# tavildar/Polar

Hardware: AMD Instinct MI355X
Metric: codewords/s (N=2048 K=1024 L=32 LLR-SCL) (higher is better)
Workload: dtype f64

## Files before the change

### polar_amd/__init__.py

```python
import ctypes as C
import os

import numpy as np

try:
    import torch
except Exception:
    torch = None

_HERE = os.path.dirname(os.path.abspath(__file__))
LIB_PATH = os.environ.get("POLAR_AMD_LIB") or os.path.join(_HERE, "libpolar_amd.so")

_dp = C.POINTER(C.c_double)
_u8p = C.POINTER(C.c_uint8)
_u16p = C.POINTER(C.c_uint16)
_u64p = C.POINTER(C.c_uint64)


ASK4_GRAY, ASK8_GRAY, ASK16_GRAY, BPSK = 1, 2, 3, 4
ASK4_SP, ASK8_SP, ASK16_SP = 5, 6, 7
CONSTELLATION_NAMES = {"bpsk": BPSK, "ask4-gray": ASK4_GRAY, "ask8-gray": ASK8_GRAY, "ask16-gray": ASK16_GRAY,
                       "ask4-sp": ASK4_SP, "ask8-sp": ASK8_SP, "ask16-sp": ASK16_SP}
_NBITS = {BPSK: 1, ASK4_GRAY: 2, ASK4_SP: 2, ASK8_GRAY: 3, ASK8_SP: 3, ASK16_GRAY: 4, ASK16_SP: 4}
RX_MLC = 0x100
# ... 203 lines not shown
            if n == -1:
                return None
            if n < 0:
                raise PolarError(f"polar_debug_mc_alive: HIP status {-n - 1}")
            a = np.zeros(max(n, 1), np.uint64)
            if int(f(self._h, which, _p(a, _u64p), n)) != n:
                raise PolarError("polar_debug_mc_alive: the count changed between two reads")
            lists.append(np.sort(a[:n]))
        return tuple(lists)

    def debug_ctl_words(self, marked=True):
        f = self._L.polar_debug_ctl_words
        f.restype = C.c_long
        f.argtypes = [C.c_void_p, C.POINTER(C.c_uint32), C.c_long, C.c_int]
        words = np.zeros(self.N, np.uint32)
        n = int(f(self._h, _p(words, C.POINTER(C.c_uint32)), self.N, 1 if marked else 0))
        if n != self.N:
            raise PolarError(f"polar_debug_ctl_words: {n}")
        return words

    @classmethod
    def from_block_length(cls, block_length, info_length, design_epsilon, crc_size=0):
        n = int(round(np.log2(block_length)))
        if (1 << n) != block_length:
            raise PolarError("block_length must be a power of two")
        return cls(n, info_length, design_epsilon, crc_size)

    @classmethod
    def from_tables(cls, num_layers, info_length, crc_size, frozen, order, crc_matrix=None):
        frozen = np.ascontiguousarray(frozen, np.uint8)
        order = np.ascontiguousarray(order, np.uint16)
# ... 760 lines not shown
```

### polar_amd/build.py

```python
import os
import shutil
import subprocess
import sys

HERE = os.path.dirname(os.path.abspath(__file__))
ROOT = os.path.dirname(HERE)
CSRC = os.path.join(HERE, "csrc")
INC = os.path.join(ROOT, "include")
LIB = os.path.join(HERE, "libpolar_amd.so")
BUILD = os.path.join(HERE, "_build")
FLAGS_LIST32 = ["-mllvm", "-amdgpu-sched-strategy=max-memory-clause", "-mllvm", "-amdgpu-use-amdgpu-trackers"] + \
               os.environ.get("POLAR_LIST32_FLAGS", "").split()
FLAGS_LAT = os.environ.get("POLAR_LAT_FLAGS", "").split()
SOURCES = [("polar_kernels.hip", ["POLAR_ED_TU=0"], "", []), ("polar_kernels.hip", ["POLAR_ED_TU=1"], ".ed", []),
           ("polar_kernels.hip", ["POLAR_ED_TU=2"], ".ed32", FLAGS_LIST32), ("polar_kernels.hip", ["POLAR_ED_TU=3"], ".lat", FLAGS_LAT),
           ("polar_kernels.hip", ["POLAR_ED_TU=4"], ".list", []),
           ("polar_kernels.hip", ["POLAR_ED_TU=5"], ".headA", []), ("polar_kernels.hip", ["POLAR_ED_TU=6"], ".headB", FLAGS_LIST32),
           ("polar_kernels.hip", ["POLAR_ED_TU=7"], ".adapt", []),
           ("polar_kernels_sc.hip", [], "", []), ("polar_kernels_p1.hip", [], "", []), ("polar_channel.hip", [], "", []),
           ("polar_construct.hip", [], "", []), ("polar_kernels_mlc.hip", [], "", []), ("polar_kernels_ga.hip", [], "", []),
           ("polar_kernels_metric.hip", [], "", []), ("polar_kernels_adapt.hip", [], "", []),
           ("polar_kernels_flip.hip", [], "", [])] + \
          [(f, [], "", []) for f in ("polar_handle.cpp", "polar_decode.cpp", "polar_hostpipe.cpp", "polar_montecarlo.cpp", "polar_multi.cpp",
                                     "polar_debug.cpp", "polar_ga.cpp", "polar_bicm.cpp", "polar_list.cpp", "polar_mlc.cpp", "polar_adaptive.cpp", "polar_flip.cpp")]
TEST_HOOK_SOURCES = ("polar_montecarlo.cpp", "polar_debug.cpp")
TEST_HOOK_KERNEL_TAGS = (".ed32", ".headB")
LIB_TEST = os.path.join(HERE, "libpolar_amd_test.so")
KNOWN_DEFS = {"POLAR_MARGIN", "POLAR_SLOTHIST", "SCLAT_PROF", "POLAR_DEV_GS32", "POLAR_DEV_ONE", "POLAR_NO_FIXED_N",
              "POLAR_NO_GUARD_INT", "POLAR_NO_COLD_HINTS", "OCC", "ED_NR", "POLAR_R1_RANK", "POLAR_R1_CHAIN"}
ARCH = os.environ.get("POLAR_ARCH", "gfx950")
_flags_ok = {}


def _probe_flags(flags):
    key = tuple(flags)
    if key not in _flags_ok:
        import tempfile
        ok = list(flags)
        with tempfile.TemporaryDirectory() as d:
            src = os.path.join(d, "probe.hip")
            open(src, "w").write("#include <hip/hip_runtime.h>\n__global__ void probe_kernel() {}\n")
            pairs = [flags[i:i + 2] for i in range(0, len(flags), 2)]
            ok = []
            for pr in pairs:
# ... 171 lines not shown
```

### polar_amd/csrc/polar_debug.cpp

```cpp
#include "polar_multi.h"
#include "polar_amd_debug.h"
#ifdef POLAR_TEST_HOOKS
#include "polar_head_plan.h"
hipError_t polar_r1_counts_read_ed32(unsigned long long *out);
hipError_t polar_r1_counts_read_head(unsigned long long *out);
#endif

extern "C" {

int polar_debug_weak_leaves(const polar_code_t *h) { return polar_get_weak_leaves(h); }

int polar_debug_set(polar_code_t *h, const char *key, long value) {
    if (!h || !key) return fail(POLAR_E_ARG, "NULL argument");
    polar_code::Knobs &k = h->knobs;
    const std::string s(key);
    if (s == "mode_override") { if (value < -1 || value > 2) return fail(POLAR_E_ARG, "mode_override must be -1 (none), 0, 1 or 2"); k.mode_override = (int)value; }
    else if (s == "sc_no_fold") k.sc_no_fold = value != 0;
    else if (s == "no_tables") k.no_tables = value != 0;
    else if (s == "no_head") k.no_head = value != 0;
    else if (s == "no_r1") k.no_r1 = value != 0;
    else if (s == "head_min_b") { if (value < 0) return fail(POLAR_E_ARG, "head_min_b must be >= 0 (0 = default)"); k.head_min_b = value; }
    else if (s == "no_fuse_front") k.no_fuse_front = value != 0;
    else if (s == "no_prefix") h->prefix_on = (value == 0);
    else if (s == "no_rccl") { k.no_rccl = value != 0; multi_release(h, false); }
    else if (s == "force_rccl") { k.force_rccl = value != 0; multi_release(h, false); }
#ifdef POLAR_TEST_HOOKS
    else if (s == "host_fail_alloc") k.host_fail_alloc = value;
    else if (s == "share_device") { k.share_device = value != 0; multi_release(h, false); }
    else if (s == "fail_device") k.fail_device = (int)value;
    else if (s == "fail_collective") k.fail_collective = (int)value;
#endif
    else if (s == "lat_max_b") k.lat_max_b = value;
    else if (s == "lat_grid") { if (value < 0) return fail(POLAR_E_ARG, "lat_grid must be >= 0 (0 = default)"); k.lat_grid = value; }
    else if (s == "lane_grid") { if (value < 0) return fail(POLAR_E_ARG, "lane_grid must be >= 0 (0 = default)"); k.lane_grid = value; }
    else if (s == "list_chunk_cw") { if (value < 0) return fail(POLAR_E_ARG, "list_chunk_cw must be >= 0"); k.list_chunk_cw = value; }
// ... 40 lines not shown
        while (P < h->N && h->frozen[P]) ++P;
        const int Q = P >= 256 ? 256 : (P < 33 ? 0 : (P < 64 ? 64 : (P < 128 ? 128 : 256)));
        const HeadPlan hp = head_plan(h->frozen.data(), h->n, Q, std::min(P, Q), h->N / 2);
        if (hp.phi_h != h->last_head_phi) return -3;
        std::vector<unsigned long long> rows2((size_t)h->last_head_b * 4);
        const size_t pitch = hp.record_words() * sizeof(unsigned long long);
        if (hipMemcpy2D(rows2.data(), 32, h->d_head_rec.p + 2 * 4, pitch, 32, (size_t)h->last_head_b, hipMemcpyDeviceToHost) != hipSuccess) return -4;
        long bad = 0;
        for (long b = 0; b < h->last_head_b; ++b) {
            unsigned long long r[4];
            for (int a = 0; a < 4; ++a) r[a] = rows2[(size_t)b * 4 + a];
            bad += head_record_ok(hp, r) ? 0 : 1;
        }
        return bad;
    }
    if (s.compare(0, 3, "r1_") == 0) {
        static const char *const names[6] = {"r1_committed", "r1_discarded", "r1_rank_tried", "r1_rank_committed", "r1_chain_tried", "r1_chain_committed"};
        for (int i = 0; i < 6; ++i) {
            if (s != names[i]) continue;
            unsigned long long c[6] = {0, 0, 0, 0, 0, 0};
            if ((h->last_head_phi ? polar_r1_counts_read_head(c) : polar_r1_counts_read_ed32(c)) != hipSuccess) return -2;
            return (long)c[i];
        }
    }
#endif
    if (s == "last_rounds") return h->last_rounds;
    if (s == "last_round_max_per_device") return h->last_round_max_per_device;
    if (s == "worker_threads_started") return h->worker_threads_started;
    if (s.compare(0, 9, "round_us_") == 0) {
        if (h->round_us.empty()) return 0;
        std::vector<long> v(h->round_us);
        if (s == "round_us_count") return (long)v.size();
        if (s == "round_us_first") return v.front();
        std::sort(v.begin(), v.end());
        if (s == "round_us_min") return v.front();
// ... 33 lines not shown
    if (ensure_device(h, dg_)) return -1;
    unsigned int count = 0;
    hipError_t e = hipMemcpy(&count, h->d_nalive.p + which, sizeof count, hipMemcpyDeviceToHost);
    if (e == hipSuccess && (size_t)count > h->d_alive[which].cap) return -(long)hipErrorInvalidValue - 1;
    const long n = std::min<long>(count, cap);
    if (e == hipSuccess && out && n > 0) e = hipMemcpy(out, h->d_alive[which].p, (size_t)n * sizeof(uint64_t), hipMemcpyDeviceToHost);
    return e == hipSuccess ? (long)count : -(long)e - 1;
}

long polar_debug_ctl_words(polar_code_t *h, uint32_t *words, long cap, int marked) {
    if (!h) return -1;
    DevGuard dg_;
    if (ensure_device(h, dg_)) return -1;
    const long n = std::min<long>(h->N, cap);
    if (words && n > 0) {
        const hipError_t e = hipMemcpy(words, marked ? h->d_ctl_r1.p : h->d_ctl.p, (size_t)n * sizeof(uint32_t), hipMemcpyDeviceToHost);
        if (e != hipSuccess) return -(long)e - 1;
    }
    return h->N;
}

}
```

### polar_amd/csrc/polar_decode.cpp

```cpp
#include "polar_host.h"
#include "polar_head_plan.h"

namespace {

int effective_mode(const polar_code *h) { return h->knobs.mode_override >= 0 ? h->knobs.mode_override : h->mode; }
long lat_resident(const polar_code *h, int gs) {
    const size_t lds = polar_decode_lat_lds_bytes(h->N, gs, h->W);
    return lds <= h->lds_per_block ? (long)h->num_cu * std::min<long>(4, (long)(h->lds_per_block / lds)) : 0;
}
bool use_sc_lat(const polar_code *h, long B) {
    return h->n <= polar_sc_lat_max_log() && polar_sc_lat_lds_bytes(h->N, (int)h->sc_lat_ops.size()) <= h->lds_per_block &&
           h->knobs.lat_max_b >= 0 && B <= (h->knobs.lat_max_b ? h->knobs.lat_max_b : 2048);
}

struct Call {
    polar_code *h;
    const void *d_llr; int llr_fmt; long B; const unsigned int *n_dev; int L; uint8_t *d_out; double *d_pm;
    hipStream_t st; void *ev_start, *ev_stop; int phase; Deferred *deferred;
    BatchGeometry g; PolarDecodeParams p;
};

int batch_setup(polar_code *h, long B, int L, BatchGeometry &g) {
    if (!batch_geometry(h, B, L, true, g)) return fail(POLAR_E_ARG, "lds_log %d does not fit the LDS", g.lds_log);
    if ((size_t)g.grid * g.big * 64 + 64 > h->d_llr_scr.cap) {
// ... 203 lines not shown
    BatchGeometry gm = *std::max_element(g, g + n, [](const BatchGeometry &a, const BatchGeometry &b) { return a.grid < b.grid; });
    int rc;
    while ((rc = ensure_batch_scratch(h, gm)) == POLAR_E_NOMEM && gm.grid > gm.wpb) {
        (void)hipGetLastError();
        gm.grid = std::max(gm.wpb, (gm.grid / 2 / gm.wpb) * gm.wpb);
    }
    for (int s = 0; s < n && !rc; ++s) g[s].grid = std::min(g[s].grid, gm.grid);
    return rc;
}

void polar_host::base_params(const polar_code *h, int L, long B, PolarDecodeParams &p) {
    p.n = h->n; p.N = h->N; p.K = h->K; p.crc = h->crc; p.L = L; p.W = h->W; p.B = B;
    p.prefix_q = 0; p.prefix_len = 0; p.pre = nullptr;
    p.llr = nullptr; p.llr_fmt = POLAR_LLR_F64; p.p0 = nullptr; p.out = nullptr; p.pm_out = nullptr;
    p.frozen = h->d_frozen.p; p.info_rank = h->d_info_rank.p; p.crc_mask = h->d_crc_mask.p; p.tabs = h->d_tabs.p;
    p.ctl = h->knobs.no_r1 ? h->d_ctl.p : h->d_ctl_r1.p; p.work = h->d_work.p; p.llr_scr = h->d_llr_scr.p; p.c_scr = h->d_c_scr.p; p.hist_scr = h->d_hist_scr.p;
    p.flags = nullptr; p.cw_list = nullptr; p.cw_count = nullptr; p.n_dev = nullptr; p.tab_scr = nullptr; p.var_scr = nullptr;
}

void polar_host::fill_enc(const polar_code *h, PolarEncodeParams &p) {
    memset(&p, 0, sizeof p);
    p.n = h->n; p.N = h->N; p.K = h->K; p.crc = h->crc;
    p.order = h->d_order.p; p.crcm = h->d_crcm.p;
    p.stride = 1;
    p.info_block_div = 100;
}

int polar_host::decode_impl(polar_code *h, const void *d_llr, int llr_fmt, long B, const unsigned int *n_dev, int L, uint8_t *d_out,
                            double *d_pm, void *stream, void *ev_start, void *ev_stop, int phase, Deferred *deferred) {
    if (deferred) *deferred = Deferred::None;
    int rc = check_args(h && d_llr && d_out, L, B);
// ... 195 lines not shown
```

### polar_amd/csrc/polar_handle.cpp

```cpp
#include "polar_host.h"

namespace polar_host {

thread_local std::string g_err;

int fail(int code, const char *fmt, ...) {
    char buf[512];
    va_list ap;
    va_start(ap, fmt);
    vsnprintf(buf, sizeof buf, fmt, ap);
    va_end(ap);
    g_err = buf;
    return code;
}

std::atomic<unsigned long> g_allocs{0};

int usable_cpus() {
    int n = (int)std::thread::hardware_concurrency();
    cpu_set_t set;
    if (sched_getaffinity(0, sizeof set, &set) == 0) n = CPU_COUNT(&set);
    if (FILE *f = fopen("/sys/fs/cgroup/cpu.max", "r")) {
        char q[32]; long per = 0;
        if (fscanf(f, "%31s %ld", q, &per) == 2 && strcmp(q, "max") != 0 && per > 0) n = std::min<long>(n, std::max<long>(1, atol(q) / per));
// ... 133 lines not shown
        std::vector<int> tu((size_t)N + 1, 0);
        for (int i = 0; i < N; ++i) tu[i + 1] = tu[i] + (h->frozen[i] ? 0 : 1);
        auto rate1 = [&](int i0, int Z) {
            if (i0 + Z > N) return false;
            for (int i = i0; i < i0 + Z; ++i) {
                if (h->frozen[i] || (h->ctl[i] & 0x100u)) return false;
                if (i < i0 + Z - 1 && (tu[i] & 31) == 31) return false;
            }
            return true;
        };
        for (int i = 0; i < N; i += 4) {
            if ((i & 7) == 0 && rate1(i, 8)) { h->ctl_r1[i] |= 3u << 9; h->ctl_r1[i + 4] |= 2u << 9; i += 4; continue; }
            if (rate1(i, 4)) h->ctl_r1[i] |= 2u << 9;
        }
    }
    h->crc_mask.assign((size_t)crc * h->W, 0u);
    for (int i = 0; i < crc; ++i) {
        uint32_t *m = &h->crc_mask[(size_t)i * h->W];
        for (int j = 0; j < K; ++j)
            if (h->crcm[(size_t)i * K + j] & 1) m[h->info_rank[j] >> 5] ^= 1u << (h->info_rank[j] & 31);
        int r = h->info_rank[K + i];
        m[r >> 5] ^= 1u << (r & 31);
    }
    return POLAR_OK;
}

int ensure_device(polar_code *h, DevGuard &dg) {
    if (h->ctx_stuck) return fail(POLAR_E_DEVICE, "an earlier multi-device round of this handle never returned: the handle accepts no further calls (create a new one)");
    int cur = -1;
    if (hipGetDevice(&cur) == hipSuccess && h->device >= 0 && cur != h->device) dg.prev = cur;
// ... 7 lines not shown
        return fail(POLAR_E_DEVICE, "no HIP device available (%s); this library has no CPU decode path",
                    e == hipSuccess ? "device count 0" : hipGetErrorString(e));
    if (h->device < 0) HIP_TRY(hipGetDevice(&h->device));
    HIP_TRY(hipSetDevice(h->device));
    hipDeviceProp_t prop;
    HIP_TRY(hipGetDeviceProperties(&prop, h->device));
    h->num_cu = prop.multiProcessorCount;
    {
        int v = 0;
        h->lds_per_block = (hipDeviceGetAttribute(&v, hipDeviceAttributeMaxSharedMemoryPerBlock, h->device) == hipSuccess && v > 0) ? (size_t)v : (size_t)64 * 1024;
    }
    int rc;
    if ((rc = upload(h->d_frozen, h->frozen))) return rc;
    if ((rc = upload(h->d_ctl, h->ctl))) return rc;
    if ((rc = upload(h->d_ctl_r1, h->ctl_r1))) return rc;
    if ((rc = upload(h->d_sc_ops, h->sc_ops))) return rc;
    if ((rc = upload(h->d_sc_lat_ops, h->sc_lat_ops))) return rc;
    if ((rc = upload(h->d_order, h->order))) return rc;
    if ((rc = upload(h->d_info_rank, h->info_rank))) return rc;
    if ((rc = upload(h->d_crc_mask, h->crc_mask))) return rc;
    if ((rc = upload(h->d_crcm, h->crcm))) return rc;
    {
        std::vector<double> t(322);
        for (int j = 0; j < 64; ++j) t[j] = j ? 2.0 * std::exp2(-(double)(64 - j) / 64.0) : 1.0;
        for (int j = 0; j <= 128; ++j) {
            t[64 + j] = 1.0 / (1.0 + (double)j / 128.0);
            t[64 + 129 + j] = std::log1p((double)j / 128.0);
        }
        if ((rc = upload(h->d_tabs, t))) return rc;
    }
    h->dev_ready = true;
    return POLAR_OK;
}

int read_env_knobs(polar_code *h) {
    auto on = [](const char *name) { const char *e = getenv(name); return e && *e && strcmp(e, "0") != 0; };
    if (const char *e = getenv("POLAR_MODE")) {
        if (!(e[0] >= '0' && e[0] <= '2' && e[1] == 0)) return fail(POLAR_E_ARG, "POLAR_MODE=%s: must be 0, 1 or 2", e);
        h->knobs.mode_override = e[0] - '0';
    }
    h->knobs.sc_no_fold = on("POLAR_SC_NO_FOLD");
    h->knobs.no_tables = on("POLAR_NO_TABLES");
    h->knobs.no_head = on("POLAR_NO_HEAD");
    h->knobs.no_r1 = on("POLAR_NO_R1");
    h->knobs.no_rccl = on("POLAR_NO_RCCL");
    h->knobs.force_rccl = on("POLAR_FORCE_RCCL");
    return POLAR_OK;
}

void drop_clones(polar_code *h) {
    if (h->multi_poisoned) return;
    for (polar_code *c : h->clones) polar_destroy(c);
    h->clones.clear();
    if (h->hpipe) for (polar_code *&c : h->hpipe->ctx) if (c) { polar_destroy(c); c = nullptr; }
}

}

extern "C" {
// ... 61 lines not shown
}

void polar_destroy(polar_code_t *h) {
    if (!h) return;
    if (h->multi_poisoned) return;
    multi_release(h, false);
    for (polar_code *c : h->clones) polar_destroy(c);
    h->clones.clear();
    hostpipe_release(h);
    DevGuard dg_;
    {
        int cur = -1;
        if (h->dev_ready && hipGetDevice(&cur) == hipSuccess && cur != h->device) dg_.prev = cur;
    }
    if (h->dev_ready) (void)hipSetDevice(h->device);
    h->d_frozen.release(); h->d_ctl.release(); h->d_ctl_r1.release(); h->d_crcm.release(); h->d_order.release(); h->d_info_rank.release();
    h->d_crc_mask.release(); h->d_tabs.release(); h->d_pre.release(); h->d_llr_scr.release(); h->d_c_scr.release(); h->d_hist_scr.release();
    h->d_in.release(); h->d_f32.release(); h->d_out.release(); h->d_bytes_a.release(); h->d_bytes_b.release();
    h->d_counter.release(); h->d_sel.release(); h->d_work.release();
    h->d_ech.release(); h->d_flags.release(); h->d_list.release(); h->d_count.release(); h->d_bicm_llr.release(); h->d_list_out.release(); h->d_metric_scr.release(); h->d_adapt_ctl.release();
    h->d_alive[0].release(); h->d_alive[1].release(); h->d_nalive.release(); h->d_mc_ctr.release();
    for (auto &sl : h->mc_slots) { sl.list[0].release(); sl.list[1].release(); }
    h->d_slot_n.release();
    if (h->pin_in) (void)hipHostFree(h->pin_in);
    if (h->pin_out) (void)hipHostFree(h->pin_out);
    h->d_flip_ops.release(); h->d_flip_i32.release(); h->d_sc_ops.release(); h->d_sc_lat_ops.release(); h->d_flag_words.release(); h->d_var_scr.release(); h->d_tab_scr.release(); h->d_head_rec.release();
    delete h;
}

int polar_get_params(const polar_code_t *h, int *n, int *N, int *K, int *crc) {
    if (!h) return fail(POLAR_E_ARG, "NULL handle");
// ... 65 lines not shown
```

### polar_amd/csrc/polar_host.h

```cpp
#pragma once
#include <hip/hip_runtime.h>

#include <dlfcn.h>
#include <sched.h>
#include <sys/mman.h>
#include <unistd.h>

#include <algorithm>
#include <atomic>
#include <chrono>
#include <condition_variable>
#include <memory>
#include <mutex>
#include <thread>
#include <cmath>
#include <cstdarg>
#include <cstdio>
#include <cstdlib>
#include <cstring>
#include <functional>
#include <numeric>
#include <string>
#include <vector>

// ... 164 lines not shown
};

struct polar_code {
    int n = 0, N = 0, K = 0, crc = 0;
    double eps = 0.0;
    std::vector<uint8_t> frozen;
    std::vector<uint16_t> order;
    std::vector<uint16_t> bitrev;
    std::vector<uint8_t> crcm;
    int W = 0;
    std::vector<uint16_t> info_rank;
    std::vector<uint32_t> crc_mask;
    std::vector<uint8_t> sched;
    std::vector<uint32_t> ctl;
    std::vector<uint32_t> ctl_r1;
    int weak_leaves = 0;
    std::vector<uint32_t> sc_ops;
    std::vector<uint32_t> sc_lat_ops;
    bool sc_fold = false;
    bool dev_ready = false;
    int device = -1, num_cu = 0;
    size_t lds_per_block = 0;
    DevBuf<uint8_t> d_frozen, d_crcm;
    DevBuf<uint16_t> d_order, d_info_rank;
    DevBuf<uint32_t> d_crc_mask, d_ctl, d_ctl_r1, d_sc_ops, d_sc_lat_ops, d_var_scr;
    DevBuf<double> d_tab_scr;
    DevBuf<unsigned long long> d_head_rec;
    int last_head_phi = 0;
    long last_head_b = 0;
    long last_lat_waves = 0;
    long last_lane_waves = 0;
    const unsigned int *fb_count = nullptr;
    const uint32_t *fb_list = nullptr;
    void *fb_stream = nullptr;
    long fb_b = 0;
    void note_fallback(const unsigned int *count, const uint32_t *list, void *st, long B) { fb_count = count; fb_list = list; fb_stream = st; fb_b = B; }
    DevBuf<unsigned int> d_flag_words;
    DevBuf<double> d_llr_scr, d_tabs, d_pre;
    DevBuf<uint32_t> d_c_scr, d_hist_scr;
    DevBuf<double> d_in;
// ... 8 lines not shown
    DevBuf<unsigned int> d_count;
    DevBuf<double> d_list_out;
    DevBuf<double> d_metric_scr;
    DevBuf<unsigned int> d_adapt_ctl;
    std::vector<uint32_t> flip_ops;
    DevBuf<uint32_t> d_flip_ops;
    DevBuf<int32_t> d_flip_i32;
    DevBuf<double> d_bicm_llr;
    int mode = 0;
    struct Knobs {
        int mode_override = -1;
        bool sc_no_fold = false;
        bool no_tables = false;
        bool no_head = false;
        bool no_r1 = false;
        long head_min_b = 0;
        bool no_fuse_front = false;
        bool no_rccl = false;
        bool force_rccl = false;
        bool share_device = false;
        int fail_device = -1;
        int fail_collective = -1;
        long multi_timeout_s = 1800;
        long multi_grace_s = 10;
        bool force_workers = false;
        int stall_device = -1;
        long stall_ms = 0;
        long lat_max_b = 0;
        long host_pipe_min_bytes = 0;
        long host_chunk_bytes = 0;
// ... 136 lines not shown
```

### polar_amd/csrc/polar_kernels.hip

```cpp
#include <hip/hip_runtime.h>
#include <stdint.h>
#include <type_traits>

#include "polar_kernels.h"
#include "polar_device.h"
#include "polar_edom.h"

#ifdef POLAR_PROFILE
#define PROF_DECL u64 prof_acc[40] = {0,0,0,0,0,0,0,0,0,0,0,0,0,0,0,0,0,0,0,0,0,0,0,0,0,0,0,0,0,0,0,0,0,0,0,0,0,0,0,0}; u64 prof_t = __builtin_readcyclecounter();
#define PROF(i) { u64 t_ = __builtin_readcyclecounter(); prof_acc[i] += t_ - prof_t; prof_t = t_; }
#define PROF_OUT if (lane == 0 && p.pm_out) { for (int i_ = 0; i_ < 40; ++i_) atomicAdd((u64 *)p.pm_out + (i_ < 32 ? i_ : i_ + 2), prof_acc[i_]); }
#define PROF_CNT(i, v) { prof_acc[i] += (u64)(v); }
#define PROF_HEAD_DECL const int prof_head_phi = p.pm_out ? (int)((const u64 *)p.pm_out)[32] : 0; const u64 prof_head_t0 = prof_t; bool prof_head_open = prof_head_phi > 0;
#define PROF_HEAD(phi_) if (prof_head_open && (phi_) >= prof_head_phi) { prof_acc[22] += __builtin_readcyclecounter() - prof_head_t0; prof_head_open = false; }
#define PROF_HEAD_END prof_acc[23] += __builtin_readcyclecounter() - prof_head_t0;
#define PROF_R1_DECL int prof_r1_left = 0, prof_r1_slot = 24; bool prof_r1_open = false; u64 prof_r1_t0 = 0; \
                     const unsigned prof_r1_sw = p.pm_out ? (unsigned)((const u64 *)p.pm_out)[33] : 0u; \
                     const bool prof_r1_off = (prof_r1_sw & 1u) != 0, prof_rank_off = (prof_r1_sw & 2u) != 0, prof_chain_off = (prof_r1_sw & 4u) != 0; \
                     (void)prof_r1_off; (void)prof_rank_off; (void)prof_chain_off;
#define PROF_R1_ADD(d_) { if (prof_r1_slot == 24) prof_acc[24] += (d_); else if (prof_r1_slot == 32) prof_acc[32] += (d_); else prof_acc[34] += (d_); }
#define PROF_R1_TOP { if (prof_r1_open) { PROF_R1_ADD(prof_t - prof_r1_t0) prof_r1_open = false; } \
                      if (prof_r1_left > 0) { prof_r1_t0 = prof_t; prof_r1_open = true; --prof_r1_left; } }
#define PROF_R1_LEAF(ctl_, fast_, full_) { const int rb_ = (int)((ctl_) >> 9) & 3; \
                      if (prof_r1_open) { if (!(fast_) && prof_r1_slot == 24) prof_acc[27] += 1; } \
                      else if (rb_) { if (fast_) { prof_acc[25] += 1; prof_r1_left = (1 << rb_) - 1; prof_r1_slot = 24; } \
                                      else { prof_acc[26] += 1; if (full_) { prof_acc[33] += 1; prof_r1_left = 3; prof_r1_slot = 32; } } } }
#define PROF_R1_COMMIT prof_r1_left = 0;
#define PROF_R1_OCTET(open_) if (open_) { prof_acc[35] += 1; prof_r1_left = 1; prof_r1_slot = 34; }
#define PROF_R1_END if (prof_r1_open) { PROF_R1_ADD(__builtin_readcyclecounter() - prof_r1_t0) prof_r1_open = false; }
#else
#define PROF_R1_DECL constexpr bool prof_r1_off = false, prof_rank_off = false, prof_chain_off = false; (void)prof_r1_off; (void)prof_rank_off; (void)prof_chain_off;
#define PROF_R1_TOP
#define PROF_R1_LEAF(ctl_, fast_, full_)
#define PROF_R1_COMMIT
#define PROF_R1_OCTET(open_)
#define PROF_R1_END
#define PROF_HEAD_DECL
#define PROF_HEAD(phi_)
#define PROF_HEAD_END
#define PROF_DECL
#define PROF(i)
#define PROF_CNT(i, v)
#define PROF_OUT
#endif

#include "polar_llr_nodes.h"
// ... 45 lines not shown
#endif
#ifndef POLAR_HEAD
#define POLAR_HEAD 0
#endif
#if defined(POLAR_ED_TU) && (POLAR_ED_TU == 2 || POLAR_ED_TU == 6) && !defined(POLAR_MARGIN)
#define POLAR_R1 1
#else
#define POLAR_R1 0
#endif
#ifndef POLAR_R1_RANK
#define POLAR_R1_RANK 1
#endif
#ifndef POLAR_R1_CHAIN
#define POLAR_R1_CHAIN 1
#endif
#if POLAR_R1 && defined(POLAR_TEST_HOOKS)
__device__ unsigned long long polar_r1_counts_dev[6];
#define R1_CNT_DECL unsigned r1_cnt[6] = {0, 0, 0, 0, 0, 0};
#define R1_CNT(i_) ++r1_cnt[i_];
#define R1_CNT_OUT if (lane == 0) { for (int i_ = 0; i_ < 6; ++i_) atomicAdd(&polar_r1_counts_dev[i_], (unsigned long long)r1_cnt[i_]); }
#else
#define R1_CNT_DECL
#define R1_CNT(i_)
#define R1_CNT_OUT
#endif
template <int GS, int LDS_LOG, int PIPE, bool ED, int NL = 0, int LAT = 0>
__global__ __launch_bounds__(PIPE ? 64 : 256, PIPE ? 2 : OCC) void scl_decode_llr_kernel(POLAR_KPARAMS p) {
    constexpr int WPB = PIPE ? 1 : 4;
    constexpr bool CH_N16 = !ED;
    constexpr int G = LAT ? 1 : 64 / GS;
    constexpr int EL = 64 / GS;
    constexpr int CST = LAT ? GS : 64;
#define POLAR_CL (LAT ? lig : lane)
#define POLAR_CGB (LAT ? 0 : gbase)
    constexpr int SL = 1 << LDS_LOG;
// ... 177 lines not shown
        auto ctl_window = [&](int w0) -> uint32_t { const int i_ = w0 + lane_id_opaque(); return p.ctl[i_ < N ? i_ : 0]; };
        uint32_t ctl_next;
        if constexpr (LAT) {
            ctlv = ctl_window(phi_start & ~63);
            ctlv_n = ctl_window((phi_start & ~63) + 64);
            ctl_next = (uint32_t)__builtin_amdgcn_readlane((int)ctlv, phi_start & 63);
        } else ctl_next = ctlp[phi_start];
#if POLAR_HEAD == 1
        for (int phi = phi_start; phi < p.head_phi; ++phi) {
#else
        for (int phi = phi_start; phi < N; ++phi) {
#endif
            PROF_HEAD(phi)
            PROF(0)
            PROF_R1_TOP
            const uint32_t ctl = ctl_next;
            auto update_c = [&](int S, uint32_t X, int ph) {
                LANE_CTX
                if constexpr (LAT) {
                    if (S == 1 && N >= 128) {
                        uint32_t lo = (uint32_t)clsmall, hi = (uint32_t)(clsmall >> 32);
                        bool done = false;
                        auto level = [&](auto SC_) {
                            constexpr int Sc = decltype(SC_)::value;
                            if (done) return;
                            const uint32_t cl = (Sc == 16) ? (lo >> 16) : ((lo >> Sc) & ((1u << Sc) - 1u));
                            const uint32_t nw = (cl ^ X) | (X << Sc);
                            if (!((ph >> 1) & 1)) {
                                if constexpr (Sc == 16) hi = nw;
                                else if constexpr (Sc == 8) lo = (lo & 0x0000FFFFu) | (nw << 16);
                                else lo = (lo & ~(((1u << (2 * Sc)) - 1u) << (2 * Sc))) | (nw << (2 * Sc));
// ... 45 lines not shown
                                }
                            };
                            if (nwd >= 8) chunk(std::integral_constant<int, 8>{});
                            else if (nwd == 4) chunk(std::integral_constant<int, 4>{});
                            else chunk(std::integral_constant<int, 2>{});
                            if (!to_right) pC.set(sh + 1, lig);
                        }
                    }
                    wave_mem_fence();
                    if (!to_right) break;
                    S *= 2;
                    ph = psi;
                }
            };
            const int zb = (int)(ctl >> 1) & 0x7F;
            {
                const int nphi = phi + (1 << zb);
                if constexpr (LAT) {
                    if (POLAR_UNLIKELY2(((nphi ^ phi) & ~63) != 0)) { ctlv = ctlv_n; ctlv_n = ctl_window((nphi & ~63) + 64); }
                    ctl_next = (uint32_t)__builtin_amdgcn_readlane((int)ctlv, nphi & 63);
                } else ctl_next = ctlp[nphi < N ? nphi : 0];
            }
#if POLAR_R1
            bool r1_done = false;
#endif
            const int lam_stop = n - zb;
#include "polar_scl_visits.inc"
#include "polar_scl_leaf.inc"
        }
        PROF_R1_END
        PROF_HEAD_END
        PROF_OUT

#if POLAR_HEAD == 1
        {
            static_assert(GS == 4 && ED && !LAT && !PIPE && LDS_LOG == 3, "export exists for the groups of 4 lanes in the default tuning");
            (void)K; (void)g_tb;
            if (valid) {
                u64 *rec = p.head_rec + (size_t)cw * (size_t)p.head_rows * 4 + lig;
                rec[0] = active ? (u64)__double_as_longlong(pm) : 0ull;
                rec[4] = clsmall;
// ... 389 lines not shown
#else
hipError_t polar_launch_decode_llr_adapt(const PolarAdaptParams &p, int gs, int grid, hipStream_t st) {
    if (!p.out || !p.ad_retry || grid < 4 || (grid & 3)) return hipErrorInvalidValue;
    return launch_finish_gs(p, gs, grid, st);
}
#endif
#elif POLAR_ED_TU == 5
hipError_t polar_launch_decode_head_export(const PolarHeadParams &p, int grid, hipStream_t st) {
    if (!p.head_rec || p.L != 4 || p.head_phi <= 0 || p.head_phi >= p.N || grid < 4 || (grid & 3)) return hipErrorInvalidValue;
    hipLaunchKernelGGL((scl_decode_llr_kernel<4, 3, 0, true>), dim3(grid / 4), dim3(256), polar_decode_lds_bytes(3, 0), st, p);
    return hipGetLastError();
}
#elif POLAR_ED_TU == 6
#ifdef POLAR_TEST_HOOKS
static hipError_t r1_counts_zero(hipStream_t st) {
    static const unsigned long long z[6] = {0, 0, 0, 0, 0, 0};
    return hipMemcpyToSymbolAsync(HIP_SYMBOL(polar_r1_counts_dev), z, sizeof z, 0, hipMemcpyHostToDevice, st);
}
hipError_t polar_r1_counts_read_head(unsigned long long *out) { return hipMemcpyFromSymbol(out, HIP_SYMBOL(polar_r1_counts_dev), 6 * sizeof(unsigned long long)); }
#endif
hipError_t polar_launch_decode_head_import(const PolarHeadParams &p, int grid, hipStream_t st) {
#ifdef POLAR_TEST_HOOKS
    if (hipError_t e = r1_counts_zero(st)) return e;
#endif
    if (!p.head_rec || p.L < 17 || p.L > 32 || p.head_phi <= 0 || p.head_phi >= p.N || grid < 4 || (grid & 3)) return hipErrorInvalidValue;
    const size_t lds = polar_decode_lds_bytes(3, 0);
#ifndef POLAR_NO_FIXED_N
    if (p.n == 11) hipLaunchKernelGGL((scl_decode_llr_kernel<32, 3, 0, true, 11>), dim3(grid / 4), dim3(256), lds, st, p);
    else if (p.n == 10) hipLaunchKernelGGL((scl_decode_llr_kernel<32, 3, 0, true, 10>), dim3(grid / 4), dim3(256), lds, st, p);
    else
#endif
    hipLaunchKernelGGL((scl_decode_llr_kernel<32, 3, 0, true>), dim3(grid / 4), dim3(256), lds, st, p);
    return hipGetLastError();
}
#elif POLAR_ED_TU == 2
#ifdef POLAR_TEST_HOOKS
hipError_t polar_r1_counts_read_ed32(unsigned long long *out) { return hipMemcpyFromSymbol(out, HIP_SYMBOL(polar_r1_counts_dev), 6 * sizeof(unsigned long long)); }
#endif
hipError_t polar_launch_decode_llr_ed1_gs32(const PolarDecodeParams &p, int lds_log, int pipe, int grid, hipStream_t st) {
#ifdef POLAR_TEST_HOOKS
    {
        static const unsigned long long z[6] = {0, 0, 0, 0, 0, 0};
        if (hipError_t e = hipMemcpyToSymbolAsync(HIP_SYMBOL(polar_r1_counts_dev), z, sizeof z, 0, hipMemcpyHostToDevice, st)) return e;
    }
#endif
    return launch_gs<32, true>(p, lds_log, pipe, grid, st);
}
#elif POLAR_ED_TU == 1
hipError_t polar_launch_decode_llr_ed1_gs32(const PolarDecodeParams &p, int lds_log, int pipe, int grid, hipStream_t st);
hipError_t polar_launch_decode_llr_ed1(const PolarDecodeParams &p, int gs, int lds_log, int pipe, int grid, hipStream_t st) {
    switch (gs) {
#ifndef POLAR_DEV_GS32
        case 4: return launch_gs<4, true>(p, lds_log, pipe, grid, st);
        case 8: return launch_gs<8, true>(p, lds_log, pipe, grid, st);
        case 16: return launch_gs<16, true>(p, lds_log, pipe, grid, st);
        case 64: return launch_gs<64, true>(p, lds_log, pipe, grid, st);
#endif
// ... 24 lines not shown
```

### polar_amd/csrc/polar_multi.cpp

```cpp
#include "polar_multi.h"

namespace polar_host {

Rccl g_rccl;
std::atomic<int> g_comm_inits{0};

void multi_release(polar_code *h, bool abort_comms) {
    MultiCtx *m = h->multi;
    if (!m) return;
    h->multi = nullptr;
    if (m->stuck) {
        for (auto &t : m->threads) t.detach();
        h->multi_poisoned = true;
        return;
    }
    m->stop_workers();
    int prev = -1;
    (void)hipGetDevice(&prev);
    for (size_t d = 0; d < m->comms.size(); ++d)
        if (void *c = m->take_comm((int)d)) {
            if (abort_comms && g_rccl.CommAbort) (void)g_rccl.CommAbort(c);
            else (void)g_rccl.CommDestroy(c);
        }
    for (size_t d = 0; d < m->streams.size(); ++d)
// ... 2 lines not shown
    delete m;
}
polar_code *clone_on_device(polar_code *h, int dev, bool fresh) {
    if (!fresh) {
        if (dev == h->device) return h;
        for (polar_code *c : h->clones) if (c->device == dev) return c;
    }
    polar_code *c = copy_ctx(h, dev);
    h->clones.push_back(c);
    return c;
}
polar_code *copy_ctx(polar_code *h, int dev) {
    polar_code *c = new polar_code;
    c->n = h->n; c->N = h->N; c->K = h->K; c->crc = h->crc; c->eps = h->eps;
    c->frozen = h->frozen; c->order = h->order; c->bitrev = h->bitrev; c->crcm = h->crcm;
    c->W = h->W; c->info_rank = h->info_rank; c->crc_mask = h->crc_mask; c->sched = h->sched; c->ctl = h->ctl; c->ctl_r1 = h->ctl_r1;
    c->sc_ops = h->sc_ops; c->sc_lat_ops = h->sc_lat_ops; c->sc_fold = h->sc_fold; c->weak_leaves = h->weak_leaves;
    c->device = dev;
    c->waves_per_cu = h->waves_per_cu; c->lds_log = h->lds_log; c->pipe = h->pipe; c->prefix_on = h->prefix_on; c->mode = h->mode;
    c->knobs = h->knobs;
    return c;
}

}
```

### polar_amd/csrc/polar_scl_leaf.inc

```
            if (zb) {
                const int Z = 1 << zb;
                LANE_CTX
                auto block4 = [&](double v0, double v1, double v2, double v3) {
                    double lf[4] = {0, 0, 0, 0};
                    if (active) {
                        double a0, a1;
                        FN2(v0, v2, v1, v3, a0, a1);
                        const double b0 = GN(v0, v2, 0u, 0), b1 = GN(v1, v3, 0u, 0);
                        FN2(a0, a1, b0, b1, lf[0], lf[2]);
                        lf[1] = GN(a0, a1, 0u, 0); lf[3] = GN(b0, b1, 0u, 0);
                    }
                    if constexpr (LAT && ED) {
                        bool ng[4]; double alz[4], sneg[4], spos[4];
                        leaf_terms_ed_block<4>(lf, actw, tb, ng, alz, sneg, spos);
#pragma unroll
                        for (int i = 0; i < 4; ++i)
                            if (active) pm += ng[i] ? spos[i] : sneg[i];
                    } else {
#pragma unroll
                    for (int i = 0; i < 4; ++i) {
                        bool ng; double alz, sneg, spos;
                        leaf_terms<ED>(lf[i], active, actw, tb, ng, alz, sneg, spos);
                        if (active) pm += ng ? spos : sneg;
                    }
// ... 460 lines not shown
                        g_hist[(size_t)w * CST + POLAR_CL] = hword;
                        g_horg[(size_t)w * CST + POLAR_CL] = (uint32_t)origin;
                        origin = lig;
                        hword = 0;
                    }
                    wave_mem_fence();
                }
                ++t;
            }

            PROF(frozen ? 5 : 6)
#if POLAR_R1
            if (r1_done) {
            } else
#endif
            if ((phi & 1) == 0) {
                if (active) clsmall = (clsmall & ~2ull) | ((u64)ubit << 1);
            } else {
                update_c(1, ubit, phi);
            }
            PROF(7)
```

Measured before the change: 1.143 million.

## Decode rate-0-prefix (repetition) subtrees of size 2-8 as a single node

Adds a control table marking aligned blocks of 2, 4 or 8 leaves in which every leaf except the last is frozen (repetition nodes). The ED list-32 SCL kernel then stops the tree descent at that block, computes the frozen-leaf path-metric terms and the last leaf's LLR directly from the parent LLRs, and writes the repeated partial-sum bits in one update. This cuts the per-leaf f/g traversal and per-phi loop overhead for these blocks. It adds register pressure and new code paths in a hot kernel, and a wrong partial-sum or metric update would corrupt decoding.

```diff
diff --git a/polar_amd/__init__.py b/polar_amd/__init__.py
--- a/polar_amd/__init__.py
+++ b/polar_amd/__init__.py
@@ -241,7 +241,7 @@
         f.restype = C.c_long
         f.argtypes = [C.c_void_p, C.POINTER(C.c_uint32), C.c_long, C.c_int]
         words = np.zeros(self.N, np.uint32)
-        n = int(f(self._h, _p(words, C.POINTER(C.c_uint32)), self.N, 1 if marked else 0))
+        n = int(f(self._h, _p(words, C.POINTER(C.c_uint32)), self.N, 2 if marked == 2 else (1 if marked else 0)))
         if n != self.N:
             raise PolarError(f"polar_debug_ctl_words: {n}")
         return words
diff --git a/polar_amd/build.py b/polar_amd/build.py
--- a/polar_amd/build.py
+++ b/polar_amd/build.py
@@ -27,7 +27,7 @@
 TEST_HOOK_KERNEL_TAGS = (".ed32", ".headB")
 LIB_TEST = os.path.join(HERE, "libpolar_amd_test.so")
 KNOWN_DEFS = {"POLAR_MARGIN", "POLAR_SLOTHIST", "SCLAT_PROF", "POLAR_DEV_GS32", "POLAR_DEV_ONE", "POLAR_NO_FIXED_N",
-              "POLAR_NO_GUARD_INT", "POLAR_NO_COLD_HINTS", "OCC", "ED_NR", "POLAR_R1_RANK", "POLAR_R1_CHAIN"}
+              "POLAR_NO_GUARD_INT", "POLAR_NO_COLD_HINTS", "OCC", "ED_NR", "POLAR_R1_RANK", "POLAR_R1_CHAIN", "POLAR_R0P"}
 ARCH = os.environ.get("POLAR_ARCH", "gfx950")
 _flags_ok = {}
 
diff --git a/polar_amd/csrc/polar_debug.cpp b/polar_amd/csrc/polar_debug.cpp
--- a/polar_amd/csrc/polar_debug.cpp
+++ b/polar_amd/csrc/polar_debug.cpp
@@ -19,6 +19,7 @@
     else if (s == "no_tables") k.no_tables = value != 0;
     else if (s == "no_head") k.no_head = value != 0;
     else if (s == "no_r1") k.no_r1 = value != 0;
+    else if (s == "no_r0p") k.no_r0p = value != 0;
     else if (s == "head_min_b") { if (value < 0) return fail(POLAR_E_ARG, "head_min_b must be >= 0 (0 = default)"); k.head_min_b = value; }
     else if (s == "no_fuse_front") k.no_fuse_front = value != 0;
     else if (s == "no_prefix") h->prefix_on = (value == 0);
@@ -89,11 +90,16 @@
         }
         return bad;
     }
+    if (s == "r0p_blocks") {
+        unsigned long long c[7] = {0, 0, 0, 0, 0, 0, 0};
+        if ((h->last_head_phi ? polar_r1_counts_read_head(c) : polar_r1_counts_read_ed32(c)) != hipSuccess) return -2;
+        return (long)c[6];
+    }
     if (s.compare(0, 3, "r1_") == 0) {
         static const char *const names[6] = {"r1_committed", "r1_discarded", "r1_rank_tried", "r1_rank_committed", "r1_chain_tried", "r1_chain_committed"};
         for (int i = 0; i < 6; ++i) {
             if (s != names[i]) continue;
-            unsigned long long c[6] = {0, 0, 0, 0, 0, 0};
+            unsigned long long c[7] = {0, 0, 0, 0, 0, 0, 0};
             if ((h->last_head_phi ? polar_r1_counts_read_head(c) : polar_r1_counts_read_ed32(c)) != hipSuccess) return -2;
             return (long)c[i];
         }
@@ -157,7 +163,7 @@
     if (ensure_device(h, dg_)) return -1;
     const long n = std::min<long>(h->N, cap);
     if (words && n > 0) {
-        const hipError_t e = hipMemcpy(words, marked ? h->d_ctl_r1.p : h->d_ctl.p, (size_t)n * sizeof(uint32_t), hipMemcpyDeviceToHost);
+        const hipError_t e = hipMemcpy(words, marked == 2 ? h->d_ctl_r0p.p : (marked ? h->d_ctl_r1.p : h->d_ctl.p), (size_t)n * sizeof(uint32_t), hipMemcpyDeviceToHost);
         if (e != hipSuccess) return -(long)e - 1;
     }
     return h->N;
diff --git a/polar_amd/csrc/polar_decode.cpp b/polar_amd/csrc/polar_decode.cpp
--- a/polar_amd/csrc/polar_decode.cpp
+++ b/polar_amd/csrc/polar_decode.cpp
@@ -241,7 +241,7 @@
     p.prefix_q = 0; p.prefix_len = 0; p.pre = nullptr;
     p.llr = nullptr; p.llr_fmt = POLAR_LLR_F64; p.p0 = nullptr; p.out = nullptr; p.pm_out = nullptr;
     p.frozen = h->d_frozen.p; p.info_rank = h->d_info_rank.p; p.crc_mask = h->d_crc_mask.p; p.tabs = h->d_tabs.p;
-    p.ctl = h->knobs.no_r1 ? h->d_ctl.p : h->d_ctl_r1.p; p.work = h->d_work.p; p.llr_scr = h->d_llr_scr.p; p.c_scr = h->d_c_scr.p; p.hist_scr = h->d_hist_scr.p;
+    p.ctl = h->knobs.no_r1 ? h->d_ctl.p : (h->knobs.no_r0p ? h->d_ctl_r1.p : h->d_ctl_r0p.p); p.work = h->d_work.p; p.llr_scr = h->d_llr_scr.p; p.c_scr = h->d_c_scr.p; p.hist_scr = h->d_hist_scr.p;
     p.flags = nullptr; p.cw_list = nullptr; p.cw_count = nullptr; p.n_dev = nullptr; p.tab_scr = nullptr; p.var_scr = nullptr;
 }
 
diff --git a/polar_amd/csrc/polar_handle.cpp b/polar_amd/csrc/polar_handle.cpp
--- a/polar_amd/csrc/polar_handle.cpp
+++ b/polar_amd/csrc/polar_handle.cpp
@@ -171,6 +171,21 @@
             if (rate1(i, 4)) h->ctl_r1[i] |= 2u << 9;
         }
     }
+    h->ctl_r0p = h->ctl_r1;
+    if (h->n >= 4) {
+        for (int phi = 0; phi < N;) {
+            int zp = 0;
+            for (int z = 3; z >= 1 && !zp; --z) {
+                const int Z = 1 << z;
+                if (phi % Z || phi + Z > N || h->frozen[phi + Z - 1]) continue;
+                bool run = true;
+                for (int i = phi; i < phi + Z - 1; ++i) run = run && h->frozen[i];
+                if (run) zp = z;
+            }
+            if (zp) { h->ctl_r0p[phi] |= (uint32_t)zp << 11; phi += 1 << zp; }
+            else ++phi;
+        }
+    }
     h->crc_mask.assign((size_t)crc * h->W, 0u);
     for (int i = 0; i < crc; ++i) {
         uint32_t *m = &h->crc_mask[(size_t)i * h->W];
@@ -208,6 +223,7 @@
     if ((rc = upload(h->d_frozen, h->frozen))) return rc;
     if ((rc = upload(h->d_ctl, h->ctl))) return rc;
     if ((rc = upload(h->d_ctl_r1, h->ctl_r1))) return rc;
+    if ((rc = upload(h->d_ctl_r0p, h->ctl_r0p))) return rc;
     if ((rc = upload(h->d_sc_ops, h->sc_ops))) return rc;
     if ((rc = upload(h->d_sc_lat_ops, h->sc_lat_ops))) return rc;
     if ((rc = upload(h->d_order, h->order))) return rc;
@@ -237,6 +253,7 @@
     h->knobs.no_tables = on("POLAR_NO_TABLES");
     h->knobs.no_head = on("POLAR_NO_HEAD");
     h->knobs.no_r1 = on("POLAR_NO_R1");
+    h->knobs.no_r0p = on("POLAR_NO_R0P");
     h->knobs.no_rccl = on("POLAR_NO_RCCL");
     h->knobs.force_rccl = on("POLAR_FORCE_RCCL");
     return POLAR_OK;
@@ -328,7 +345,7 @@
         if (h->dev_ready && hipGetDevice(&cur) == hipSuccess && cur != h->device) dg_.prev = cur;
     }
     if (h->dev_ready) (void)hipSetDevice(h->device);
-    h->d_frozen.release(); h->d_ctl.release(); h->d_ctl_r1.release(); h->d_crcm.release(); h->d_order.release(); h->d_info_rank.release();
+    h->d_frozen.release(); h->d_ctl.release(); h->d_ctl_r1.release(); h->d_ctl_r0p.release(); h->d_crcm.release(); h->d_order.release(); h->d_info_rank.release();
     h->d_crc_mask.release(); h->d_tabs.release(); h->d_pre.release(); h->d_llr_scr.release(); h->d_c_scr.release(); h->d_hist_scr.release();
     h->d_in.release(); h->d_f32.release(); h->d_out.release(); h->d_bytes_a.release(); h->d_bytes_b.release();
     h->d_counter.release(); h->d_sel.release(); h->d_work.release();
diff --git a/polar_amd/csrc/polar_host.h b/polar_amd/csrc/polar_host.h
--- a/polar_amd/csrc/polar_host.h
+++ b/polar_amd/csrc/polar_host.h
@@ -202,6 +202,7 @@
     std::vector<uint8_t> sched;
     std::vector<uint32_t> ctl;
     std::vector<uint32_t> ctl_r1;
+    std::vector<uint32_t> ctl_r0p;
     int weak_leaves = 0;
     std::vector<uint32_t> sc_ops;
     std::vector<uint32_t> sc_lat_ops;
@@ -211,7 +212,7 @@
     size_t lds_per_block = 0;
     DevBuf<uint8_t> d_frozen, d_crcm;
     DevBuf<uint16_t> d_order, d_info_rank;
-    DevBuf<uint32_t> d_crc_mask, d_ctl, d_ctl_r1, d_sc_ops, d_sc_lat_ops, d_var_scr;
+    DevBuf<uint32_t> d_crc_mask, d_ctl, d_ctl_r1, d_ctl_r0p, d_sc_ops, d_sc_lat_ops, d_var_scr;
     DevBuf<double> d_tab_scr;
     DevBuf<unsigned long long> d_head_rec;
     int last_head_phi = 0;
@@ -250,6 +251,7 @@
         bool no_tables = false;
         bool no_head = false;
         bool no_r1 = false;
+        bool no_r0p = false;
         long head_min_b = 0;
         bool no_fuse_front = false;
         bool no_rccl = false;
diff --git a/polar_amd/csrc/polar_kernels.hip b/polar_amd/csrc/polar_kernels.hip
--- a/polar_amd/csrc/polar_kernels.hip
+++ b/polar_amd/csrc/polar_kernels.hip
@@ -7,9 +7,9 @@
 #include "polar_edom.h"
 
 #ifdef POLAR_PROFILE
-#define PROF_DECL u64 prof_acc[40] = {0,0,0,0,0,0,0,0,0,0,0,0,0,0,0,0,0,0,0,0,0,0,0,0,0,0,0,0,0,0,0,0,0,0,0,0,0,0,0,0}; u64 prof_t = __builtin_readcyclecounter();
+#define PROF_DECL u64 prof_acc[42] = {0,0,0,0,0,0,0,0,0,0,0,0,0,0,0,0,0,0,0,0,0,0,0,0,0,0,0,0,0,0,0,0,0,0,0,0,0,0,0,0,0,0}; u64 prof_t = __builtin_readcyclecounter();
 #define PROF(i) { u64 t_ = __builtin_readcyclecounter(); prof_acc[i] += t_ - prof_t; prof_t = t_; }
-#define PROF_OUT if (lane == 0 && p.pm_out) { for (int i_ = 0; i_ < 40; ++i_) atomicAdd((u64 *)p.pm_out + (i_ < 32 ? i_ : i_ + 2), prof_acc[i_]); }
+#define PROF_OUT if (lane == 0 && p.pm_out) { for (int i_ = 0; i_ < 42; ++i_) atomicAdd((u64 *)p.pm_out + (i_ < 32 ? i_ : i_ + 2), prof_acc[i_]); }
 #define PROF_CNT(i, v) { prof_acc[i] += (u64)(v); }
 #define PROF_HEAD_DECL const int prof_head_phi = p.pm_out ? (int)((const u64 *)p.pm_out)[32] : 0; const u64 prof_head_t0 = prof_t; bool prof_head_open = prof_head_phi > 0;
 #define PROF_HEAD(phi_) if (prof_head_open && (phi_) >= prof_head_phi) { prof_acc[22] += __builtin_readcyclecounter() - prof_head_t0; prof_head_open = false; }
@@ -17,7 +17,10 @@
 #define PROF_R1_DECL int prof_r1_left = 0, prof_r1_slot = 24; bool prof_r1_open = false; u64 prof_r1_t0 = 0; \
                      const unsigned prof_r1_sw = p.pm_out ? (unsigned)((const u64 *)p.pm_out)[33] : 0u; \
                      const bool prof_r1_off = (prof_r1_sw & 1u) != 0, prof_rank_off = (prof_r1_sw & 2u) != 0, prof_chain_off = (prof_r1_sw & 4u) != 0; \
-                     (void)prof_r1_off; (void)prof_rank_off; (void)prof_chain_off;
+                     const bool prof_r0p_off = (prof_r1_sw & 8u) != 0; int prof_r0p_end = -1; u64 prof_r0p_t0 = 0; \
+                     (void)prof_r1_off; (void)prof_rank_off; (void)prof_chain_off; (void)prof_r0p_off; (void)prof_r0p_end; (void)prof_r0p_t0;
+#define PROF_R0P_TOP(phi_) if ((phi_) == prof_r0p_end) { prof_acc[40] += prof_t - prof_r0p_t0; prof_r0p_end = -1; }
+#define PROF_R0P_SKIP(phi_, Z_) { prof_acc[41] += 1; prof_r0p_end = (phi_) + (Z_) - 1; prof_r0p_t0 = prof_t; }
 #define PROF_R1_ADD(d_) { if (prof_r1_slot == 24) prof_acc[24] += (d_); else if (prof_r1_slot == 32) prof_acc[32] += (d_); else prof_acc[34] += (d_); }
 #define PROF_R1_TOP { if (prof_r1_open) { PROF_R1_ADD(prof_t - prof_r1_t0) prof_r1_open = false; } \
                       if (prof_r1_left > 0) { prof_r1_t0 = prof_t; prof_r1_open = true; --prof_r1_left; } }
@@ -29,7 +32,10 @@
 #define PROF_R1_OCTET(open_) if (open_) { prof_acc[35] += 1; prof_r1_left = 1; prof_r1_slot = 34; }
 #define PROF_R1_END if (prof_r1_open) { PROF_R1_ADD(__builtin_readcyclecounter() - prof_r1_t0) prof_r1_open = false; }
 #else
-#define PROF_R1_DECL constexpr bool prof_r1_off = false, prof_rank_off = false, prof_chain_off = false; (void)prof_r1_off; (void)prof_rank_off; (void)prof_chain_off;
+#define PROF_R1_DECL constexpr bool prof_r1_off = false, prof_rank_off = false, prof_chain_off = false, prof_r0p_off = false; \
+                     (void)prof_r1_off; (void)prof_rank_off; (void)prof_chain_off; (void)prof_r0p_off;
+#define PROF_R0P_TOP(phi_)
+#define PROF_R0P_SKIP(phi_, Z_)
 #define PROF_R1_TOP
 #define PROF_R1_LEAF(ctl_, fast_, full_)
 #define PROF_R1_COMMIT
@@ -105,11 +111,18 @@
 #ifndef POLAR_R1_CHAIN
 #define POLAR_R1_CHAIN 1
 #endif
+#ifndef POLAR_R0P
+#define POLAR_R0P 1
+#endif
+#if !POLAR_R1
+#undef POLAR_R0P
+#define POLAR_R0P 0
+#endif
 #if POLAR_R1 && defined(POLAR_TEST_HOOKS)
-__device__ unsigned long long polar_r1_counts_dev[6];
-#define R1_CNT_DECL unsigned r1_cnt[6] = {0, 0, 0, 0, 0, 0};
+__device__ unsigned long long polar_r1_counts_dev[7];
+#define R1_CNT_DECL unsigned r1_cnt[7] = {0, 0, 0, 0, 0, 0, 0};
 #define R1_CNT(i_) ++r1_cnt[i_];
-#define R1_CNT_OUT if (lane == 0) { for (int i_ = 0; i_ < 6; ++i_) atomicAdd(&polar_r1_counts_dev[i_], (unsigned long long)r1_cnt[i_]); }
+#define R1_CNT_OUT if (lane == 0) { for (int i_ = 0; i_ < 7; ++i_) atomicAdd(&polar_r1_counts_dev[i_], (unsigned long long)r1_cnt[i_]); }
 #else
 #define R1_CNT_DECL
 #define R1_CNT(i_)
@@ -317,7 +330,12 @@
             PROF_HEAD(phi)
             PROF(0)
             PROF_R1_TOP
+            PROF_R0P_TOP(phi)
+#if POLAR_R0P
+            uint32_t ctl = ctl_next;
+#else
             const uint32_t ctl = ctl_next;
+#endif
             auto update_c = [&](int S, uint32_t X, int ph) {
                 LANE_CTX
                 if constexpr (LAT) {
@@ -393,8 +411,20 @@
                 }
             };
             const int zb = (int)(ctl >> 1) & 0x7F;
+#if POLAR_R0P
+            int zs = zb;
+            int r0p_z = 0;
+            if constexpr (ED && !LAT && GS == 32) {
+                int zp = (int)(ctl >> 11) & 3;
+                if (LDS_LOG < 3 && zp == 3) zp = 0;
+                if (zp && prof_r0p_off) { PROF_R0P_SKIP(phi, 1 << zp) zp = 0; }
+                if (zp) zs = zp;
+            }
+#else
+            const int zs = zb;
+#endif
             {
-                const int nphi = phi + (1 << zb);
+                const int nphi = phi + (1 << zs);
                 if constexpr (LAT) {
                     if (POLAR_UNLIKELY2(((nphi ^ phi) & ~63) != 0)) { ctlv = ctlv_n; ctlv_n = ctl_window((nphi & ~63) + 64); }
                     ctl_next = (uint32_t)__builtin_amdgcn_readlane((int)ctlv, nphi & 63);
@@ -403,7 +433,7 @@
 #if POLAR_R1
             bool r1_done = false;
 #endif
-            const int lam_stop = n - zb;
+            const int lam_stop = n - zs;
 #include "polar_scl_visits.inc"
 #include "polar_scl_leaf.inc"
         }
@@ -823,10 +853,10 @@
 #elif POLAR_ED_TU == 6
 #ifdef POLAR_TEST_HOOKS
 static hipError_t r1_counts_zero(hipStream_t st) {
-    static const unsigned long long z[6] = {0, 0, 0, 0, 0, 0};
+    static const unsigned long long z[7] = {0, 0, 0, 0, 0, 0, 0};
     return hipMemcpyToSymbolAsync(HIP_SYMBOL(polar_r1_counts_dev), z, sizeof z, 0, hipMemcpyHostToDevice, st);
 }
-hipError_t polar_r1_counts_read_head(unsigned long long *out) { return hipMemcpyFromSymbol(out, HIP_SYMBOL(polar_r1_counts_dev), 6 * sizeof(unsigned long long)); }
+hipError_t polar_r1_counts_read_head(unsigned long long *out) { return hipMemcpyFromSymbol(out, HIP_SYMBOL(polar_r1_counts_dev), 7 * sizeof(unsigned long long)); }
 #endif
 hipError_t polar_launch_decode_head_import(const PolarHeadParams &p, int grid, hipStream_t st) {
 #ifdef POLAR_TEST_HOOKS
@@ -844,12 +874,12 @@
 }
 #elif POLAR_ED_TU == 2
 #ifdef POLAR_TEST_HOOKS
-hipError_t polar_r1_counts_read_ed32(unsigned long long *out) { return hipMemcpyFromSymbol(out, HIP_SYMBOL(polar_r1_counts_dev), 6 * sizeof(unsigned long long)); }
+hipError_t polar_r1_counts_read_ed32(unsigned long long *out) { return hipMemcpyFromSymbol(out, HIP_SYMBOL(polar_r1_counts_dev), 7 * sizeof(unsigned long long)); }
 #endif
 hipError_t polar_launch_decode_llr_ed1_gs32(const PolarDecodeParams &p, int lds_log, int pipe, int grid, hipStream_t st) {
 #ifdef POLAR_TEST_HOOKS
     {
-        static const unsigned long long z[6] = {0, 0, 0, 0, 0, 0};
+        static const unsigned long long z[7] = {0, 0, 0, 0, 0, 0, 0};
         if (hipError_t e = hipMemcpyToSymbolAsync(HIP_SYMBOL(polar_r1_counts_dev), z, sizeof z, 0, hipMemcpyHostToDevice, st)) return e;
     }
 #endif
diff --git a/polar_amd/csrc/polar_multi.cpp b/polar_amd/csrc/polar_multi.cpp
--- a/polar_amd/csrc/polar_multi.cpp
+++ b/polar_amd/csrc/polar_multi.cpp
@@ -40,7 +40,7 @@
     polar_code *c = new polar_code;
     c->n = h->n; c->N = h->N; c->K = h->K; c->crc = h->crc; c->eps = h->eps;
     c->frozen = h->frozen; c->order = h->order; c->bitrev = h->bitrev; c->crcm = h->crcm;
-    c->W = h->W; c->info_rank = h->info_rank; c->crc_mask = h->crc_mask; c->sched = h->sched; c->ctl = h->ctl; c->ctl_r1 = h->ctl_r1;
+    c->W = h->W; c->info_rank = h->info_rank; c->crc_mask = h->crc_mask; c->sched = h->sched; c->ctl = h->ctl; c->ctl_r1 = h->ctl_r1; c->ctl_r0p = h->ctl_r0p;
     c->sc_ops = h->sc_ops; c->sc_lat_ops = h->sc_lat_ops; c->sc_fold = h->sc_fold; c->weak_leaves = h->weak_leaves;
     c->device = dev;
     c->waves_per_cu = h->waves_per_cu; c->lds_log = h->lds_log; c->pipe = h->pipe; c->prefix_on = h->prefix_on; c->mode = h->mode;
diff --git a/polar_amd/csrc/polar_scl_leaf.inc b/polar_amd/csrc/polar_scl_leaf.inc
--- a/polar_amd/csrc/polar_scl_leaf.inc
+++ b/polar_amd/csrc/polar_scl_leaf.inc
@@ -1,3 +1,61 @@
+#if POLAR_R0P
+            if (zs != zb) {
+                const int zp = zs;
+                const uint32_t ctl_last = ctlp[phi + (1 << zp) - 1];
+                const int Z = 1 << zp;
+                LANE_CTX
+                auto term = [&](double v) {
+                    bool ng; double alz, sneg, spos;
+                    leaf_terms<ED>(v, active, actw, tb, ng, alz, sneg, spos);
+                    if (active) pm += ng ? spos : sneg;
+                };
+                auto quad = [&](double v0, double v1, double v2, double v3, int nm) -> double {
+                    double lf[4] = {0, 0, 0, 0};
+                    if (active) {
+                        double a0, a1;
+                        FN2(v0, v2, v1, v3, a0, a1);
+                        const double b0 = GN(v0, v2, 0u, 0), b1 = GN(v1, v3, 0u, 0);
+                        FN2(a0, a1, b0, b1, lf[0], lf[2]);
+                        lf[1] = GN(a0, a1, 0u, 0); lf[3] = GN(b0, b1, 0u, 0);
+                    }
+#pragma unroll
+                    for (int i = 0; i < 3; ++i) term(lf[i]);
+                    if (nm == 4) term(lf[3]);
+                    return lf[3];
+                };
+                const double *yp = lds_llr + (size_t)(Z - 1) * 64 + lane;
+                if (zp == 1) {
+                    double y0 = 0, y1 = 0, l0 = 0;
+                    if (active) { y0 = yp[0]; y1 = yp[64]; l0 = FN(y0, y1); leaf = GN(y0, y1, 0u, 0); }
+                    term(l0);
+                } else if (zp == 2) {
+                    double y[4] = {0, 0, 0, 0};
+                    if (active) {
+#pragma unroll
+                        for (int j = 0; j < 4; ++j) y[j] = yp[(size_t)j * 64];
+                    }
+                    leaf = quad(y[0], y[1], y[2], y[3], 3);
+                } else {
+                    double a[4] = {0, 0, 0, 0}, b[4] = {0, 0, 0, 0};
+                    if (active) {
+#pragma unroll
+                        for (int j = 0; j < 4; ++j) {
+                            const double lo = yp[(size_t)j * 64], hi = yp[(size_t)(j + 4) * 64];
+                            a[j] = FN(lo, hi);
+                            b[j] = GN(lo, hi, 0u, 0);
+                        }
+                    }
+                    quad(a[0], a[1], a[2], a[3], 4);
+                    leaf = quad(b[0], b[1], b[2], b[3], 3);
+                }
+                R1_CNT(6)
+                PROF_CNT(41, 1)
+                PROF(5)
+                phi += Z - 1;
+                ctl = ctl_last;
+                r0p_z = zp;
+            } else
+#endif
             if (zb) {
                 const int Z = 1 << zb;
                 LANE_CTX
@@ -498,6 +556,20 @@
             if (r1_done) {
             } else
 #endif
+#if POLAR_R0P
+            if (r0p_z) {
+                const int zp = r0p_z;
+                const int Z = 1 << zp;
+                const uint32_t X = ubit ? ((1u << Z) - 1u) : 0u;
+                const int nu = phi >> zp;
+                if ((nu & 1) == 0) {
+                    if (active) clsmall = (clsmall & ~((((u64)1 << Z) - 1ull) << Z)) | ((u64)X << Z);
+                } else {
+                    update_c(Z, X, nu);
+                }
+                wave_mem_fence();
+            } else
+#endif
             if ((phi & 1) == 0) {
                 if (active) clsmall = (clsmall & ~2ull) | ((u64)ubit << 1);
             } else {
```

Measured after the change: 1.155 million (median of 6 runs). About the same (+1.0%).
